# ConwayBeyond/Funscript-Flow

Hardware: AMD Instinct MI355X
Metric: 1080p frame-pairs/sec (higher is better)
Workload: dtype f32; 1 GPU; 1920x1080 synthetic sine-translate frame-pair stream, gray frames resident in HBM; levels=4, winsize=15, poly_n=5, parallelism=pair-shard x1, compute_lanes=1, kernel_signature=872b792e378b97e5

## Files before the change

### funscript_flow_amd/csrc/ffl_api.hip

```cpp
#include "../../include/ffl.h"
#include "ffl_kernels.h"

#include <math.h>
#include <stdarg.h>
#include <stdio.h>
#include <string.h>

#include <algorithm>
#include <condition_variable>
#include <mutex>
#include <string>
#include <thread>
#include <vector>

#define FFL_EV_RING 16
#define FFL_RAW_RING 4

template <class H, class Arg, hipError_t (*Free)(Arg)>
struct Owned {
    H h = H();
    Owned() = default;
    explicit Owned(H take) : h(take) {}
    Owned(Owned &&o) noexcept : h(o.release()) {}
    Owned &operator=(Owned &&o) noexcept { std::swap(h, o.h); return *this; }
// ... 1254 lines not shown
    HIPCHK(c, hipStreamSynchronize(c->s_copy));
    return FFL_OK;
}

struct DebugCapture {
    int level, iter;
    float *I0, *I1, *R0, *R1, *M, *flow;
};

static int enqueue_batch(ffl_ctx *c, ffl_ctx::Lane &L, const BatchTab &T, int n, int nU, int pov_mode, const DebugCapture *cap) {
    hipStream_t st = L.st;
    const size_t N = c->N;
    const UTab *ut = &L.d_tab->ut;
    const PairTab *pt = &L.d_tab->pt;
    const PyrJob *l0 = &L.pyr[L.n_jobs - 1];
    const bool fuse_l0 = c->opt.fuse_l0_blur && ffl_polyexp_from_gray_ok(*l0);
    const int skip_l0 = fuse_l0 && !cap;
    {
        ProfScope ps(c, FFL_K_PYRAMID, st);
        if (!ffl_launch_pyr_multi(c->d_gray, N, ut, nU, L.pyr, L.n_jobs - skip_l0, c->opt, st))
            for (int k = c->geo.levels; k >= skip_l0; k--)
                ffl_launch_pyr_level(c->d_gray, N, ut, nU, L.pyr[c->geo.levels - k], st);
    }
    {
        ProfScope ps(c, FFL_K_POLYEXP, st);
        ffl_launch_polyexp_multi(L.poly, L.n_jobs, nU, c->pc, c->d_gray, N, ut, fuse_l0 ? l0 : nullptr, st);
    }

    int pw = 0, ph = 0;
    for (int k = c->geo.levels; k >= 0; k--) {
        const LevelGeom &g = c->geo.lv[k];
        const int lw = g.lw, lh = g.lh;
        const size_t plane = (size_t)lw * lh;
        const size_t I_stride = plane, R_stride = 5 * plane, M_stride = 5 * plane;
        float *Rk = L.d_R + c->lay.r_off[k];
        if (pw == 0 && cap)
            for (int i = 0; i < n; i++) HIPCHK(c, hipMemsetAsync(T.pt.flow[k][i], 0, sizeof(float) * 2 * plane, st));
        int mi = 0;
        const bool fuse_first = c->opt.fuse_first > 0 && !cap && (long)((lw + 63) / 64) * ((lh + 15) / 16) * n >= c->opt.fuse_first;
        if (!fuse_first) {
            ProfScope ps(c, FFL_K_UPDATE_MATRICES, st);
            ffl_launch_update_matrices(Rk, R_stride, plane, pt, k, n, L.d_M[mi], M_stride, lw, lh, pw, ph, pw == 0, cap != nullptr, c->opt, st);
        }
        bool captured = false;
        auto capture = [&]() -> int {
            HIPCHK(c, hipStreamSynchronize(st));
            if (cap->I0) HIPCHK(c, hipMemcpy(cap->I0, L.d_I + c->lay.i_off[k] + (size_t)T.pt.u0[0] * I_stride, sizeof(float) * plane, hipMemcpyDeviceToHost));
            if (cap->I1) HIPCHK(c, hipMemcpy(cap->I1, L.d_I + c->lay.i_off[k] + (size_t)T.pt.u1[0] * I_stride, sizeof(float) * plane, hipMemcpyDeviceToHost));
            if (cap->R0) HIPCHK(c, hipMemcpy(cap->R0, Rk + (size_t)T.pt.u0[0] * R_stride, sizeof(float) * 5 * plane, hipMemcpyDeviceToHost));
            if (cap->R1) HIPCHK(c, hipMemcpy(cap->R1, Rk + (size_t)T.pt.u1[0] * R_stride, sizeof(float) * 5 * plane, hipMemcpyDeviceToHost));
            if (cap->M) HIPCHK(c, hipMemcpy(cap->M, L.d_M[mi], sizeof(float) * 5 * plane, hipMemcpyDeviceToHost));
            if (cap->flow) HIPCHK(c, hipMemcpy(cap->flow, T.pt.flow[k][0], sizeof(float) * 2 * plane, hipMemcpyDeviceToHost));
            captured = true;
            return FFL_OK;
        };
        for (int it = 0; it < 3; it++) {
            if (cap && cap->level == k && cap->iter == it) {
                int rc = capture();
                if (rc) return rc;
            }
            const int update = it < 2;
            {
                ProfScope ps(c, FFL_K_BLUR_SOLVE, st, it > 0 && !cap);
                if (it == 0 && fuse_first)
                    ffl_launch_blur_solve_first(L.d_M[mi ^ 1], M_stride, Rk, R_stride, plane, pt, k, n, lw, lh, pw, ph, c->opt, c->blur_slots, st);
                else
                    ffl_launch_blur_solve(L.d_M[mi], L.d_M[mi ^ 1], M_stride, Rk, R_stride, plane, pt, k, n, lw, lh,
                                          update, cap != nullptr, c->opt, c->blur_slots, st);
            }
            if (update) mi ^= 1;
        }
        if (cap && cap->level == k && !captured) {
            int rc = capture();
            if (rc) return rc;
        }
        pw = lw;
        ph = lh;
    }
    {
        ProfScope ps(c, FFL_K_PASS1, st);
        ffl_launch_pass1(pt, n, c->w, c->h, pov_mode, L.d_pkey, L.d_psum, st);
    }
    return FFL_OK;
}

static int batch_graph(ffl_ctx *c, ffl_ctx::Lane &L, const BatchTab &T, int n, int nU, int pov_mode,
                       ffl_ctx::Lane::GraphEntry **ge) {
    *ge = nullptr;
    for (auto &g : L.graphs)
        if (g.n == n && g.nU == nU && g.pov == pov_mode && g.epoch == c->opt_epoch) *ge = &g;
    if (*ge || c->graph_bad_epoch == c->opt_epoch) return FFL_OK;
    hipStream_t st = L.st;
    ffl_ctx::Lane::GraphEntry g = {n, nU, pov_mode, c->opt_epoch, Graph(), GraphExec()};
    hipError_t fail = hipStreamBeginCapture(st, hipStreamCaptureModeThreadLocal);
    if (fail == hipSuccess) {
        const int rc = enqueue_batch(c, L, T, n, nU, pov_mode, nullptr);
        fail = hipStreamEndCapture(st, g.graph.put());
        if (fail == hipSuccess && (rc != FFL_OK || !g.graph)) fail = hipErrorStreamCaptureInvalidated;
        if (fail == hipSuccess) fail = hipGraphInstantiate(g.exec.put(), g.graph, nullptr, nullptr, 0);
    }
    if (fail != hipSuccess) {
        g.exec.reset();
        g.graph.reset();
        (void)hipGetLastError();
// ... 41 lines not shown
        const size_t plane = (size_t)c->geo.lv[k].lw * c->geo.lv[k].lh;
        float *buf = ((c->geo.levels - k) & 1) ? L.d_flowB : L.d_flowA;
        for (int i = 0; i < n; i++)
            T.pt.flow[k][i] = (k == 0) ? c->d_flow + (size_t)slots[i] * 2 * N : buf + (size_t)i * 2 * plane;
    }
    for (int k = c->geo.levels + 1; k < FFL_MAX_LEVELS; k++)
        for (int i = 0; i < n; i++) T.pt.flow[k][i] = nullptr;
    for (int i = 0; i < nU; i++) c->u_of_fslot[T.ut.fslot[i]] = -1;
    *nU_out = nU;
    WaitOnce wait(st);
    for (int i = 0; i < nU; i++) HIPCHK(c, wait(c->ev_uploaded[T.ut.fslot[i]].get()));
    for (int i = 0; i < n; i++) HIPCHK(c, wait(c->ev_slot_done[slots[i]].get()));
    HIPCHK(c, hipMemcpyAsync(L.d_tab, &T, sizeof(BatchTab), hipMemcpyHostToDevice, st));

    if (fbg || dis) {
        if (fbg) {
            FbgWork wk;
            if (int rc = fbg_work(c, L, *fbg, nU, &wk)) return rc;
            ffl_launch_fb_general(&L.d_tab->ut, &L.d_tab->pt, n, nU, c->d_gray, N, c->w, c->h, *fbg, wk, st);
        } else {
            ffl_launch_dis(&L.d_tab->ut, &L.d_tab->pt, n, c->d_gray, N, L.d_M[0], *dis, st);
        }
        ProfScope ps(c, FFL_K_PASS1, st);
        ffl_launch_pass1(&L.d_tab->pt, n, c->w, c->h, pov_mode, L.d_pkey, L.d_psum, st);
    } else if (c->opt.use_graph && !cap && c->prof_mask == 0) {
        ffl_ctx::Lane::GraphEntry *ge;
        if (int rc = batch_graph(c, L, T, n, nU, pov_mode, &ge)) return rc;
        if (ge) {
            HIPCHK(c, hipGraphLaunch(ge->exec, st));
            c->graph_replayed++;
        } else if (int rc = enqueue_batch(c, L, T, n, nU, pov_mode, nullptr)) {
            return rc;
        }
    } else if (int rc = enqueue_batch(c, L, T, n, nU, pov_mode, cap)) {
        return rc;
    }
    HIPCHK(c, hipGetLastError());
    return FFL_OK;
}

static int run_batch(ffl_ctx *c, int li, int n, const int *f0, const int *f1, const int *slots, int pov_mode,
                     const DebugCapture *cap, const DisKParams *dis = nullptr, const FbgPlan *fbg = nullptr) {
    ffl_ctx::Lane &L = c->lanes[li];
    HIPCHK(c, L.ring.settle_next());
    BatchTab &T = L.h_tab[L.ring.next % FFL_EV_RING];
    int nU = 0;
    const int rc = queue_batch(c, L, T, &nU, n, f0, f1, slots, pov_mode, cap, dis, fbg);
// ... 1952 lines not shown
    if (int rc = check_flow_slots(c, fn, n, dst_slots, nullptr, "repeated among the dst slots of one call")) return rc;
    int clash = -1;
    for (int i = 0; i < n; i++) c->slot_mark[src_slots[i]] = 1;
    for (int i = 0; i < n; i++)
        if (c->slot_mark[dst_slots[i]] && dst_slots[i] != src_slots[i] && clash < 0) clash = dst_slots[i];
    for (int i = 0; i < n; i++) c->slot_mark[src_slots[i]] = 0;
    if (clash >= 0) return set_err(c, FFL_ERR_INVALID, "%s: dst flow slot %d is another item's src slot", fn, clash);
    if (!models_dev) return set_err(c, FFL_ERR_INVALID, "%s: NULL models_dev", fn);
    if (int rc = model_array_check(c, fn, "models_dev", models_dev, model_stride)) return rc;
    int all[2 * FFL_MAXB], m = 0;
    ExportTab ts, td;
    for (int i = 0; i < n; i++) all[m++] = ts.slot[i] = src_slots[i];
    for (int i = 0; i < n; i++) {
        td.slot[i] = dst_slots[i];
        if (dst_slots[i] != src_slots[i]) all[m++] = dst_slots[i];
    }
    hipStream_t cst;
    const PostRegion reg{"models_dev", models_dev, (size_t)(n - 1) * (size_t)model_stride + 48, kHostModels};
    if (int rc = post_begin(c, fn, stream, &cst, &reg, 1, m, all)) return rc;
    ffl_launch_motion_subtract(c->d_flow, c->d_res, ts, td, n, c->w, c->h, (const char *)models_dev, (long long)model_stride, c->d_ptab,
                               c->s_post);
    {
        ProfScope ps(c, FFL_K_PASS1, c->s_post);
        ffl_launch_pass1(c->d_ptab, n, c->w, c->h, pov_mode ? 1 : 0, c->d_pskey, c->d_rpsum, c->s_post);
    }
    return post_end(c, cst, m, all);
}

static int dev_flow_check(ffl_ctx *c, const char *fn, int dtype, int n, int w, int h, const ffl_dev_flow *f, int *mode,
                          size_t *bytes) {
    if (!f) return set_err(c, FFL_ERR_INVALID, "%s: NULL descriptor", fn);
    if (dtype != FFL_F32 && dtype != FFL_F16 && dtype != FFL_BF16)
        return set_err(c, FFL_ERR_INVALID, "%s: unknown dtype %d (FFL_F32 0, FFL_F16 1, FFL_BF16 2)", fn, dtype);
    if (n < 1) return set_err(c, FFL_ERR_INVALID, "%s: n = %d fields (>= 1)", fn, n);
    if (w < 2 || h < 2 || w > 32768 || h > 32768) return set_err(c, FFL_ERR_INVALID, "%s: size %dx%d outside 2..32768", fn, w, h);
    if (!f->base) return set_err(c, FFL_ERR_INVALID, "%s: NULL base", fn);
    const ptrdiff_t e = dtype == FFL_F32 ? 4 : 2, big = (ptrdiff_t)1 << 40;
    const ptrdiff_t it = f->item_stride, pitch = f->row_pitch, ps = f->pixel_stride, cs = f->channel_stride;
    if (it < 0 || pitch < 0 || ps < 0 || cs < 0)
        return set_err(c, FFL_ERR_INVALID, "%s: negative stride (item %td, row %td, pixel %td, channel %td)", fn, it, pitch, ps, cs);
    if (it > big || pitch > big || ps > big || cs > big) return set_err(c, FFL_ERR_INVALID, "%s: stride beyond 2^40", fn);
    if ((uintptr_t)f->base % e || it % e || pitch % e || ps % e || cs % e)
        return set_err(c, FFL_ERR_INVALID, "%s: misaligned: base and strides (item %td, row %td, pixel %td, channel %td) must be "
                                           "multiples of the element size %td", fn, it, pitch, ps, cs, e);
    if (ps < e) return set_err(c, FFL_ERR_INVALID, "%s: overlap: pixel stride %td below the element size %td", fn, ps, e);
    const ptrdiff_t row = (ptrdiff_t)(w - 1) * ps + e, plane = (ptrdiff_t)(h - 1) * pitch + row;
    if (pitch < row) return set_err(c, FFL_ERR_INVALID, "%s: overlap: row pitch %td too small for %d pixels %td bytes apart", fn, pitch, w, ps);
// ... 35 lines not shown
                                c->s_post);
    }
    return post_end(c, cst, n, slots);
}

int ffl_upload_flow(ffl_ctx *c, int slot, const float *src, int pov_mode) {
    if (!c) return FFL_ERR_INVALID;
    std::unique_lock<std::mutex> pl(c->post_mu);
    CtxLock lk(c->mu);
    if (!flow_slot_ok(c, slot) || !src) return set_err(c, FFL_ERR_INVALID, "ffl_upload_flow: bad arguments");
    hipStream_t st = c->s_post;
    hipEvent_t ev = c->ev_slot_done[slot].get();
    if (int rc = wait_unlocked(c, lk, &ev, 1)) return rc;
    lk.unlock();
    hipError_t se = hipStreamSynchronize(st);
    lk.lock();
    HIPCHK(c, se);
    HIPCHK(c, hipMemcpy(c->d_flow + (size_t)slot * 2 * c->N, src, sizeof(float) * 2 * c->N, hipMemcpyHostToDevice));
    c->h_ptab->flow[0][0] = c->d_flow + (size_t)slot * 2 * c->N;
    c->h_ptab->res[0] = c->d_res + slot;
    HIPCHK(c, hipMemcpyAsync(c->d_ptab, c->h_ptab, sizeof(PairTab), hipMemcpyHostToDevice, st));
    {
        ProfScope ps(c, FFL_K_PASS1, st);
        ffl_launch_pass1(c->d_ptab, 1, c->w, c->h, pov_mode, c->d_pskey, c->d_rpsum, st);
    }
    EvRef done;
    if (int rc = publish_post(c, 1, &slot, &done)) return rc;
    HIPCHK(c, hipGetLastError());
    return FFL_OK;
}

int ffl_submit_pair(ffl_ctx *c, int slot, const uint8_t *prev, const uint8_t *next, int width, int height, int channels,
                    ptrdiff_t stride_bytes, int pov_mode) {
    if (!c) return FFL_ERR_INVALID;
    if (!flow_slot_ok(c, slot) || 2 * slot + 1 >= c->n_fslots) {
        CtxLock lk(c->mu);
        return set_err(c, FFL_ERR_INVALID, "ffl_submit_pair: slot %d needs frame slots %d,%d and a flow slot", slot, 2 * slot, 2 * slot + 1);
    }
    int rc = ffl_upload_frame(c, 2 * slot, prev, width, height, channels, stride_bytes);
    if (rc) return rc;
    rc = ffl_upload_frame(c, 2 * slot + 1, next, width, height, channels, stride_bytes);
    if (rc) return rc;
    int f0 = 2 * slot, f1 = 2 * slot + 1;
    return ffl_flow_pairs(c, 1, &f0, &f1, &slot, pov_mode);
}

int ffl_sync(ffl_ctx *c) {
// ... 138 lines not shown
```

### funscript_flow_amd/csrc/ffl_kernels.h

```cpp
#pragma once
#include <hip/hip_runtime.h>
#include <limits.h>
#include <stdint.h>

#define FFL_MAXB 256
#define FFL_MAXU (2 * FFL_MAXB)
#define FFL_MAX_LEVELS 4
#define FFL_POLY_N 5
#define FFL_WIN 15
#define FFL_WIN_R 7

struct PolyConsts {
    float g[FFL_POLY_N + 1], xg[FFL_POLY_N + 1], xxg[FFL_POLY_N + 1];
    double gd[FFL_POLY_N + 1], xxgd[FFL_POLY_N + 1];
    double ig11, ig03, ig33, ig55;
};

struct GaussKernel {
    float k[32];
    int ksize;
};

struct UTab {
    int fslot[FFL_MAXU];
// ... 87 lines not shown
    int w, h;
    unsigned gx, gy, first, count;
    int from_gray;
    float gk0, gk1;
};
struct PolyJobs {
    PolyJob j[FFL_MAX_JOBS];
    int n;
};

struct FflOptions {
    int lanes = 2;
    int fuse_first = 10000;
    int use_graph = 1;
    int copy_threads = 4;
    int blur_rows = 0;
    int blur_min_wgs = 3500;
    int tile_order = 0;
    int blur_taper = 1;
    int blur_taper_pairs = 0;
    int pyr_coarse = 1;
    int fuse_l0_blur = 1;
    int fb_general = 0;
};
struct FflOptionRow {
    const char *name;
    int FflOptions::*member;
    int lo, hi;
    bool flag;
};
inline constexpr FflOptionRow kFflOptionRows[] = {
    {"lanes", &FflOptions::lanes, 1, 4, false},
    {"fuse_first", &FflOptions::fuse_first, 0, INT_MAX, false},
    {"graph", &FflOptions::use_graph, INT_MIN, INT_MAX, true},
    {"copy_threads", &FflOptions::copy_threads, 1, 16, false},
    {"blur_rows", &FflOptions::blur_rows, 0, 64, false},
    {"blur_min_wgs", &FflOptions::blur_min_wgs, 1, INT_MAX, false},
    {"tile_order", &FflOptions::tile_order, 0, 1, false},
    {"blur_taper", &FflOptions::blur_taper, 0, 1, false},
    {"blur_taper_pairs", &FflOptions::blur_taper_pairs, 0, FFL_MAXB, false},
    {"pyr_coarse", &FflOptions::pyr_coarse, INT_MIN, INT_MAX, true},
    {"fuse_l0_blur", &FflOptions::fuse_l0_blur, INT_MIN, INT_MAX, true},
    {"fb_general", &FflOptions::fb_general, 0, 1, false},
};

#define FFL_BLUR_SEGS 3
struct BlurSeg {
    int first_block, first_pair, pairs, nrb, strips;
};
struct BlurPlan {
    BlurSeg s[FFL_BLUR_SEGS];
    int n;
};
struct BlurSlots {
    int first, first_zero, update, last;
};

bool ffl_launch_pyr_multi(const uint8_t *gray_base, size_t gray_stride, const UTab *ut, int nU, const PyrJob *levels, int n,
                          const FflOptions &opt, hipStream_t st);
bool ffl_polyexp_from_gray_ok(const PyrJob &l0);
void ffl_launch_polyexp_multi(const PolyJob *levels, int n, int nU, PolyConsts pc, const uint8_t *gray_base, size_t gray_stride,
                              const UTab *ut, const PyrJob *l0, hipStream_t st);
void ffl_launch_frontend(const FrameDesc &d, uint8_t *gray, const FrontParams &p, hipStream_t st);
void ffl_launch_frontend_dev(const FrameDesc *tab, int n, uint8_t *gray_base, size_t N, const FrontParams &p, hipStream_t st);
void ffl_launch_frontend_remap(const FrameDesc &d, uint8_t *gray, const FrontParams &p, const RemapParams &r, hipStream_t st);
void ffl_launch_frontend_remap_dev(const FrameDesc *tab, int n, uint8_t *gray_base, size_t N, const FrontParams &p,
                                   const RemapParams &r, hipStream_t st);
void ffl_launch_export_flows(const float *flow, const ExportTab &tab, int n, size_t N, char *dst, long long item_stride,
                             int layout, hipStream_t st);
void ffl_launch_import_pass1(const ImportArgs &a, const ExportTab &tab, int n, int dtype, int mode, int w, int h, int pov_mode,
                             PairTab *pt, unsigned long long *pkey, double *psum, hipStream_t st);
void ffl_launch_gray(const uint8_t *bgr, uint8_t *gray, int n_pixels, hipStream_t st);
size_t ffl_pyr_tmp_floats(int w, int h, int lw);
bool ffl_pyr_level_ok(int w, int h, int lw, int lh, int ksize);
void ffl_launch_pyr_level(const uint8_t *gray_base, size_t gray_stride, const UTab *ut, int nU, const PyrJob &level,
                          hipStream_t st);
void ffl_launch_update_matrices(const float *R, size_t R_stride, size_t plane, const PairTab *pt, int level, int nB, float *M,
                                size_t M_stride, int lw, int lh, int pw, int ph, int zero_flow, int store_flow,
                                const FflOptions &opt, hipStream_t st);
void ffl_launch_blur_solve(const float *Min, float *Mout, size_t M_stride, const float *R, size_t R_stride,
                           size_t plane, const PairTab *pt, int level, int nB, int lw, int lh, int update, int store_flow,
                           const FflOptions &opt, const BlurSlots &slots, hipStream_t st);


void ffl_launch_blur_solve_first(float *Mout, size_t M_stride, const float *R, size_t R_stride, size_t plane,
                                 const PairTab *pt, int level, int nB, int lw, int lh, int pw, int ph, const FflOptions &opt,
                                 const BlurSlots &slots, hipStream_t st);
bool ffl_blur_slots(BlurSlots *out);
unsigned ffl_blur_plan(int tiles_x, int tiles_y, int nB, int slots, const FflOptions &opt, BlurPlan *plan);

#define DIS_MAX_PATCHES 4096
#define DIS_MAX_SCALES 12
struct DisKParams {
    int w, h, finest, coarsest, stride, gd_iters, vr_iters, mean_norm, spatial_prop, stripes;
    float alpha, gamma, delta;
    size_t pair_floats;
    size_t pyr_floats;
    size_t pyr_off[DIS_MAX_SCALES];
    float *dbg;
    int dbg_scale, dbg_stage;
};
void ffl_launch_dis(const UTab *ut, const PairTab *pt, int nB, const uint8_t *gray, size_t gray_stride, float *scratch,
                    const DisKParams &p, hipStream_t st);

int ffl_pass1_blocks(int w, int h);
void ffl_launch_pass1(const PairTab *pt, int nB, int w, int h, int pov_mode, unsigned long long *pkey, double *psum,
                      hipStream_t st);

#define FFL_WINDOW_MAX_RADIUS 32
struct WindowSeq {
    int slot[FFL_MAXB + 2 * FFL_WINDOW_MAX_RADIUS];
};
struct WindowItem {
    const float *flow;
    double cx, cy;
    int cut, pad;
};
struct Pass2Record {
    double dot, cx, cy;
    float mean_mag, div_val;
    int x, y, cut, pad;
};
struct AxesRecord {
    Pass2Record base;
    double tangential, shift_x, shift_y, reserved;
};
#define FFL_NAXES 4
int ffl_radial_blocks(int w, int h);
struct RadialForm {
    int nc;
// ... 244 lines not shown
    return ffl_tile_map(blockIdx.x, tiles_x, tiles_y, nB, order, b, tile_x, tile_y);
}

__host__ __device__ __forceinline__ bool ffl_blur_block(const BlurPlan &p, unsigned blk, int tiles_x, int order, int &b,
                                                        int &tile_x, int &row0, int &nrb) {
    int first = 0, pair0 = 0, pairs = p.s[0].pairs, strips = p.s[0].strips;
    nrb = p.s[0].nrb;
#pragma unroll
    for (int i = 1; i < FFL_BLUR_SEGS; i++)
        if (i < p.n && blk >= (unsigned)p.s[i].first_block) {
            first = p.s[i].first_block;
            pair0 = p.s[i].first_pair;
            pairs = p.s[i].pairs;
            strips = p.s[i].strips;
            nrb = p.s[i].nrb;
        }
    int strip_y;
    if (!ffl_tile_map(blk - first, tiles_x, strips, pairs, order, b, tile_x, strip_y)) return false;
    b += pair0;
    row0 = strip_y * nrb;
    return true;
}

#define FFL_GLOBAL __attribute__((address_space(1)))
typedef float ffl_v2f __attribute__((ext_vector_type(2), aligned(4)));
typedef float ffl_v4f __attribute__((ext_vector_type(4), aligned(4)));
__device__ __forceinline__ float2 ffl_gload2(const void *base, size_t byte_off) {
    const ffl_v2f v = *(const FFL_GLOBAL ffl_v2f *)((const char *)base + byte_off);
    return make_float2(v.x, v.y);
}
__device__ __forceinline__ float4 ffl_gload4(const void *base, size_t byte_off) {
    const ffl_v4f v = *(const FFL_GLOBAL ffl_v4f *)((const char *)base + byte_off);
    return make_float4(v.x, v.y, v.z, v.w);
}

struct __attribute__((packed, aligned(4))) ffl_f2u { float x, y; };
struct __attribute__((packed, aligned(4))) ffl_f4u { float x, y, z, w; };

template <typename T>
__device__ __forceinline__ const T *ffl_at(const float *base, unsigned idx) {
    return reinterpret_cast<const T *>(reinterpret_cast<const char *>(base) + idx * 4u);
}
template <typename T>
__device__ __forceinline__ T *ffl_at(float *base, unsigned idx) {
    return reinterpret_cast<T *>(reinterpret_cast<char *>(base) + idx * 4u);
}
// ... 90 lines not shown
```

### funscript_flow_amd/csrc/kernels_farneback.hip

```cpp
#include "ffl_kernels.h"

#include <algorithm>

__global__ __launch_bounds__(256) void k_gray(const uint8_t *__restrict__ bgr, uint8_t *__restrict__ gray, int n) {
    int i4 = (blockIdx.x * 256 + threadIdx.x) * 4;
    if (i4 + 3 < n) {
        const uint32_t *p = reinterpret_cast<const uint32_t *>(bgr + (size_t)i4 * 3);
        uint32_t a = p[0], b = p[1], c = p[2];
        uint32_t px[12] = {a & 255, (a >> 8) & 255, (a >> 16) & 255, a >> 24, b & 255, (b >> 8) & 255,
                           (b >> 16) & 255, b >> 24, c & 255, (c >> 8) & 255, (c >> 16) & 255, c >> 24};
        uint32_t o = 0;
#pragma unroll
        for (int j = 0; j < 4; j++) {
            uint32_t g = (px[j * 3] * 3735u + px[j * 3 + 1] * 19235u + px[j * 3 + 2] * 9798u + 16384u) >> 15;
            o |= g << (8 * j);
        }
        *reinterpret_cast<uint32_t *>(gray + i4) = o;
    } else {
        for (int i = i4; i < n; i++) {
            uint32_t b = bgr[(size_t)i * 3], g = bgr[(size_t)i * 3 + 1], r = bgr[(size_t)i * 3 + 2];
            gray[i] = (uint8_t)((b * 3735u + g * 19235u + r * 9798u + 16384u) >> 15);
        }
    }
}
// ... 685 lines not shown
                    if (x + e < w) out[c * plane + off + e] = o[c][e];
        }
    }
}

__global__ __launch_bounds__(256) void k_polyexp_multi(PolyJobs jobs, PolyConsts pc, const uint8_t *__restrict__ gray_base,
                                                       size_t gray_stride, const UTab *__restrict__ ut) {
    int i = 0;
#pragma unroll
    for (int t = 1; t < FFL_MAX_JOBS; t++)
        if (t < jobs.n && blockIdx.x >= jobs.j[t].first) i = t;
    const PolyJob &J = jobs.j[i];
    const unsigned t = blockIdx.x - J.first;
    if (t >= J.count) return;
    const unsigned per = J.gx * J.gy;
    const unsigned bz = t / per, r = t - bz * per, by = r / J.gx, bx = r - by * J.gx;
    const uint8_t *gimg = J.from_gray ? gray_base + (size_t)ut->fslot[bz] * gray_stride : nullptr;
    k_polyexp_body(bx, by, bz, J.I, J.I_stride, J.R, J.R_stride, J.plane, J.w, J.h, pc, gimg, J.gk0, J.gk1);
}

bool ffl_polyexp_from_gray_ok(const PyrJob &l0) { return ffl_pyr_form(l0.w, l0.h, l0.lw, l0.lh, l0.gk.ksize).kind == FFL_PYR_F1; }

void ffl_launch_polyexp_multi(const PolyJob *jobs_in, int n, int nU, PolyConsts pc, const uint8_t *gray_base, size_t gray_stride,
                              const UTab *ut, const PyrJob *l0, hipStream_t st) {
    PolyJobs jobs = {};
    unsigned total = 0;
    for (int i = 0; i < n; i++) {
        jobs.j[i] = jobs_in[i];
        jobs.j[i].gx = (jobs_in[i].w + PE_TW - 1) / PE_TW;
        jobs.j[i].gy = (jobs_in[i].h + PE_TH - 1) / PE_TH;
        jobs.j[i].first = total;
        jobs.j[i].count = jobs.j[i].gx * jobs.j[i].gy * (unsigned)nU;
        total += jobs.j[i].count;
    }
    jobs.n = n;
    if (l0) {
        jobs.j[n - 1].from_gray = 1;
        jobs.j[n - 1].gk0 = l0->gk.k[1];
        jobs.j[n - 1].gk1 = l0->gk.k[2];
    }
    hipLaunchKernelGGL(k_polyexp_multi, dim3(total), dim3(256), 0, st, jobs, pc, gray_base, gray_stride, ut);
}

__device__ __forceinline__ float2 ffl_upsample2(const float4 c0, const float4 c1, bool first0, bool first1, float a1, float b1) {
    const float a0 = 1.f - a1, b0 = 1.f - b1;
    const float2 p00 = first0 ? make_float2(c0.x, c0.y) : make_float2(c0.z, c0.w);
    const float2 p01 = first1 ? make_float2(c0.x, c0.y) : make_float2(c0.z, c0.w);
    const float2 p10 = first0 ? make_float2(c1.x, c1.y) : make_float2(c1.z, c1.w);
    const float2 p11 = first1 ? make_float2(c1.x, c1.y) : make_float2(c1.z, c1.w);
    float2 f;
    float t0 = p00.x * a0 + p01.x * a1, t1 = p10.x * a0 + p11.x * a1;
    f.x = (t0 * b0 + t1 * b1) * 2.0f;
    t0 = p00.y * a0 + p01.y * a1;
    t1 = p10.y * a0 + p11.y * a1;
    f.y = (t0 * b0 + t1 * b1) * 2.0f;
    return f;
}

template <int NR, typename Disp, typename Keep>
__device__ __forceinline__ void ffl_um_rows(const float *R0, const float *R1, float *M, size_t plane, int w, int h, int x,
                                            bool xin, int ybase, Disp disp, Keep keep) {
    struct UmRow {
// ... 27 lines not shown
        if (k + 1 < NR) nxt = issue(k + 1);
        const bool in = xin && ybase + 4 * k < h;
        const int y = min(ybase + 4 * k, h - 1);
        const unsigned o = (unsigned)y * (unsigned)w + (unsigned)x;
        if (in) keep(o, cur.f);
        float bb[5];
#pragma unroll
        for (int c = 0; c < 5; c++) bb[c] = cur.a00 * cur.t[c].x + cur.a01 * cur.t[c].y + cur.a10 * cur.u[c].x + cur.a11 * cur.u[c].y;
        float m[5];
        ffl_um_finish(cur.r0, bb, cur.inside, w, h, x, y, cur.f.x, cur.f.y, m);
        if (in) {
#pragma unroll
            for (int c = 0; c < 5; c++) *ffl_at<float>(M + c * plane, o) = m[c];
        }
        if (k + 1 < NR) cur = nxt;
    }
}

template <int MODE>
__global__ __launch_bounds__(256) void k_update_matrices(const float *__restrict__ R, size_t R_stride, size_t plane,
                                                         const PairTab *__restrict__ pt, int level,
                                                         float *__restrict__ M, size_t M_stride, int w,
                                                         int h, int pw, int ph, double usx, double usy, int store_flow,
                                                         int nB, int order) {
    int b, tile_x, tile_y;
    if (!ffl_tile_coord((w + 63) / 64, (h + 15) / 16, nB, order, b, tile_x, tile_y)) return;
    const int lx = threadIdx.x & 63, x0 = tile_x * 64, x = min(x0 + lx, w - 1);
    const bool xin = x0 + lx < w;
    const float *R0 = R + (size_t)pt->u0[b] * R_stride, *R1 = R + (size_t)pt->u1[b] * R_stride;
    float *flow = pt->flow[level][b];
    const float *pf = pt->flow[min(level + 1, FFL_MAX_LEVELS - 1)][b];
    constexpr int NR = 4;
    const int ybase = tile_y * 16 + (threadIdx.x >> 6);
    float2 f[NR];
    if (MODE == 1) {
        const bool half_scale = usx == 0.5 && usy == 0.5;
        int xa0, xa1;
        float a1;
        if (half_scale) ffl_resize_coord_half(x, pw, xa0, xa1, a1);
        else ffl_resize_coord(x, pw, usx, xa0, xa1, a1);
        const int xq = min(xa0, pw - 2);
        float4 c0[NR], c1[NR];
        float b1[NR];
#pragma unroll
        for (int k = 0; k < NR; k++) {
            int ya0, ya1;
            const int y = min(ybase + 4 * k, h - 1);
            if (half_scale) ffl_resize_coord_half(y, ph, ya0, ya1, b1[k]);
            else ffl_resize_coord(y, ph, usy, ya0, ya1, b1[k]);
// ... 4 lines not shown
        for (int k = 0; k < NR; k++) f[k] = ffl_upsample2(c0[k], c1[k], xa0 == xq, xa1 == xq, a1, b1[k]);
    } else if (MODE == 0) {
#pragma unroll
        for (int k = 0; k < NR; k++) {
            const unsigned o = (unsigned)min(ybase + 4 * k, h - 1) * (unsigned)w + (unsigned)x;
            const FFL_GLOBAL float *q = (const FFL_GLOBAL float *)flow + 2u * o;
            f[k] = make_float2(q[0], q[1]);
        }
    } else {
#pragma unroll
        for (int k = 0; k < NR; k++) f[k] = make_float2(0.f, 0.f);
    }
    ffl_um_rows<NR>(R0, R1, M + (size_t)b * M_stride, plane, w, h, x, xin, ybase, [&](int k) { return f[k]; },
                    [&](unsigned o, float2 d) {
                        if (MODE == 1 && store_flow) {
                            flow[2u * o] = d.x;
                            flow[2u * o + 1u] = d.y;
                        }
                    });
}

void ffl_launch_update_matrices(const float *R, size_t R_stride, size_t plane, const PairTab *pt, int level, int nB,
                                float *M,
                                size_t M_stride, int lw, int lh, int pw, int ph, int zero_flow, int store_flow,
                                const FflOptions &opt, hipStream_t st) {
    dim3 grid(ffl_tile_grid((lw + 63) / 64, (lh + 15) / 16, nB));
    const auto k = pw > 0 ? k_update_matrices<1> : (zero_flow ? k_update_matrices<2> : k_update_matrices<0>);
    hipLaunchKernelGGL(k, grid, dim3(256), 0, st, R, R_stride, plane, pt, level, M, M_stride, lw, lh, pw, ph,
                       pw > 0 ? (double)pw / lw : 1.0, pw > 0 ? (double)ph / lh : 1.0, pw > 0 ? store_flow : 0, nB,
                       opt.tile_order);
}

#ifndef FFL_K5_WAVES
#define FFL_K5_WAVES 4
#endif
#ifndef FFL_K5_WAVES_FIRST
#define FFL_K5_WAVES_FIRST 3
#endif
#ifndef FFL_K5_GROUP_FIRST
#define FFL_K5_GROUP_FIRST 3
#endif
#ifndef FFL_K5_GROUP
#define FFL_K5_GROUP 3
#endif

__device__ __forceinline__ void ffl_box_block16(const float (&v)[30], double (&out)[16]) {
    double s[15];
    s[14] = (double)v[14];
#pragma unroll
    for (int j = 13; j >= 0; j--) s[j] = (double)v[j] + s[j + 1];
    double p = (double)v[15];
    out[0] = s[0];
#pragma unroll
// ... 37 lines not shown
#define FFL_DRAIN_MAX 8192
__device__ unsigned long long g_drain[3][FFL_DRAIN_MAX][2];
extern "C" int ffl_debug_read_drain(unsigned long long *out) {
    return (int)hipMemcpyFromSymbol(out, HIP_SYMBOL(g_drain), sizeof(unsigned long long) * 3 * FFL_DRAIN_MAX * 2);
}
#define FFL_DRAIN(e)                                                          \
    if (w >= 1024 && tid == 0 && blockIdx.x < FFL_DRAIN_MAX) g_drain[FIRST ? 0 : UPDATE ? 1 : 2][blockIdx.x][e] = wall_clock64();
#define FFL_T(i)                                                              \
    if (FFL_STAMP_ON && tid == 0) {                                           \
        const unsigned long long t_ = __builtin_readcyclecounter();          \
        sStamp[i] += t_ - sStamp[FFL_NSTAMP];                                 \
        sStamp[FFL_NSTAMP] = t_;                                              \
    }
#else
#define FFL_T(i)
#define FFL_DRAIN(e)
#endif


template <bool UPDATE, int FIRST>
__global__ __launch_bounds__(256, FIRST ? FFL_K5_WAVES_FIRST : FFL_K5_WAVES) void k_blur_solve(
    const float *__restrict__ Min, float *__restrict__ Mout, size_t M_stride, const float *__restrict__ R, size_t R_stride,
    size_t plane, const PairTab *__restrict__ pt, int level, int w, int h, BlurPlan plan, int pw, int ph, double usx, double usy,
    int store_flow, int order) {
    constexpr int TW = 64, TH = 16, LW = TW + 2 * FFL_WIN_R, LH = TH + 2 * FFL_WIN_R;
    constexpr int PX = 4;
    constexpr int NCARRY = LH - TH;
    constexpr int LW2 = 44;
    constexpr int GC = FIRST ? FFL_K5_GROUP_FIRST : FFL_K5_GROUP, NG = (5 + GC - 1) / GC;
    __shared__ double2 sS2[GC][TH][LW2];
    const int tid = threadIdx.x;
#ifdef FFL_STAMP
    __shared__ unsigned long long sStamp[FFL_NSTAMP + 1];
    const bool FFL_STAMP_ON = FIRST == 1 && w >= 1024;
    if (FFL_STAMP_ON && tid == 0) {
        for (int i = 0; i < FFL_NSTAMP; i++) sStamp[i] = 0;
        sStamp[FFL_NSTAMP] = __builtin_readcyclecounter();
    }
#endif
    int b, tile_x, row0, nrb;
    if (!ffl_blur_block(plan, blockIdx.x, (w + TW - 1) / TW, order, b, tile_x, row0, nrb)) return;
    FFL_DRAIN(0)
    const int x0 = tile_x * TW;
    const float *Mb = Min + (size_t)b * M_stride;

    const int q = __builtin_amdgcn_readfirstlane(tid >> 6);
    const int ty = (tid & 63) >> 2, kk = tid & 3;
    const int lx0 = 16 * kk + 4 * q;
    double *sS = reinterpret_cast<double *>(&sS2[0][0][0]);
    const int vcc = tid / LW, vtx = tid - vcc * LW;
    const int vgx = min(max(x0 + vtx - FFL_WIN_R, 0), w - 1);
    const unsigned pitch = (unsigned)w * 4u;
    float carry[NG][NCARRY];
    const double scale = 1.0 / (FFL_WIN * FFL_WIN);
    float2 *flow = reinterpret_cast<float2 *>(pt->flow[level][b]);
    const float *R0 = R + (size_t)pt->u0[b] * R_stride, *R1 = R + (size_t)pt->u1[b] * R_stride;
    float *Mo = Mout + (size_t)b * M_stride;
    constexpr int FP = TW + 2;
    float4 *sF4 = reinterpret_cast<float4 *>(&sS2[0][0][0]);
    constexpr int UP = 80;
    __shared__ float sM34[FIRST ? 5 - GC : 1][FIRST ? TH : 1][FIRST ? UP : 1];
    float *sM012 = reinterpret_cast<float *>(&sS2[0][0][0]);
    static_assert(GC * TH * UP * 4 <= (int)sizeof(sS2), "the first group's staged rows must fit the column sums");
    const float2 *prevf = reinterpret_cast<const float2 *>(pt->flow[min(level + 1, FFL_MAX_LEVELS - 1)][b]);
// ... 268 lines not shown
    int per_cu = 0;
    if (hipOccupancyMaxActiveBlocksPerMultiprocessor(&per_cu, k, 256, 0) != hipSuccess) return 0;
    return per_cu * cus;
}
bool ffl_blur_slots(BlurSlots *out) {
    int dev = 0, cus = 0;
    if (hipGetDevice(&dev) != hipSuccess || hipDeviceGetAttribute(&cus, hipDeviceAttributeMultiprocessorCount, dev) != hipSuccess)
        return false;
    *out = BlurSlots{ffl_k5_slots(k_blur_solve<true, 1>, cus), ffl_k5_slots(k_blur_solve<true, 2>, cus),
                     ffl_k5_slots(k_blur_solve<true, 0>, cus), ffl_k5_slots(k_blur_solve<false, 0>, cus)};
    return out->first > 0 && out->first_zero > 0 && out->update > 0 && out->last > 0;
}
#ifdef FFL_STAMP
extern "C" int ffl_debug_blur_slots(int *out) {
    BlurSlots s;
    if (!ffl_blur_slots(&s)) return 1;
    out[0] = s.first; out[1] = s.first_zero; out[2] = s.update; out[3] = s.last;
    return 0;
}
#endif

template <typename K>
static void ffl_launch_k5(K k, const float *Min, float *Mout, size_t M_stride, const float *R, size_t R_stride, size_t plane,
                          const PairTab *pt, int level, int nB, int lw, int lh, int pw, int ph, int store_flow,
                          const FflOptions &opt, int slots, hipStream_t st) {
    BlurPlan plan;
    dim3 grid(ffl_blur_plan((lw + 63) / 64, (lh + 15) / 16, nB, slots, opt, &plan));
    hipLaunchKernelGGL(k, grid, dim3(256), 0, st, Min, Mout, M_stride, R, R_stride, plane, pt, level, lw, lh, plan, pw, ph,
                       pw > 0 ? (double)pw / lw : 1.0, pw > 0 ? (double)ph / lh : 1.0, store_flow, opt.tile_order);
}

void ffl_launch_blur_solve(const float *Min, float *Mout, size_t M_stride, const float *R, size_t R_stride,
                           size_t plane, const PairTab *pt, int level, int nB, int lw, int lh, int update, int store_flow,
                           const FflOptions &opt, const BlurSlots &slots, hipStream_t st) {
    ffl_launch_k5(update ? k_blur_solve<true, 0> : k_blur_solve<false, 0>, Min, Mout, M_stride, R, R_stride, plane, pt, level,
                  nB, lw, lh, 0, 0, update ? store_flow : 1, opt, update ? slots.update : slots.last, st);
}

void ffl_launch_blur_solve_first(float *Mout, size_t M_stride, const float *R, size_t R_stride, size_t plane,
                                 const PairTab *pt, int level, int nB, int lw, int lh, int pw, int ph, const FflOptions &opt,
                                 const BlurSlots &slots, hipStream_t st) {
    ffl_launch_k5(pw > 0 ? k_blur_solve<true, 1> : k_blur_solve<true, 2>, (const float *)nullptr, Mout, M_stride, R, R_stride,
                  plane, pt, level, nB, lw, lh, pw, ph, 0, opt, pw > 0 ? slots.first : slots.first_zero, st);
}
```

### funscript_flow_amd/csrc/kernels_post.hip

```cpp
#include "ffl_kernels.h"
#include <cassert>
#include <cfloat>
#include <type_traits>

#define P1_THREADS 256
#define P1_RG 16
#ifndef P1_G
#define P1_G 16
#endif
#define P1_STRIP 126
#define P2_STRIP 128
#ifndef P2_AXES_G
#define P2_AXES_G 2
#endif

static inline int ffl_strip_waves(int w, int h, int strip) {
    return ((w + strip - 1) / strip) * ((h + P1_RG - 1) / P1_RG);
}
int ffl_pass1_blocks(int w, int h) { return (ffl_strip_waves(w, h, P1_STRIP) + 3) / 4; }
int ffl_radial_blocks(int w, int h) { return (ffl_strip_waves(w, h, P2_STRIP) + 3) / 4; }

__device__ __forceinline__ float ffl_grad(float lo, float hi, int idx, int n) {
    return (idx == 0 || idx == n - 1) ? hi - lo : (hi - lo) / 2.0f;
}
// ... 129 lines not shown
    key = ffl_wave_max_u64(key);
    sum = ffl_wave_sum_f64(sum);
    if constexpr (Wt::on) sw = ffl_wave_sum_f64(sw);
    if (lane == 0) {
        skey[wv] = key;
        ssum[wv] = sum;
        if constexpr (Wt::on) ssw[wv] = sw;
    }
    __syncthreads();
    if (threadIdx.x == 0) {
        for (int i = 1; i < P1_THREADS / 64; i++) {
            key = skey[i] > key ? skey[i] : key;
            sum += ssum[i];
            if constexpr (Wt::on) sw += ssw[i];
        }
        pkey[(size_t)b * gridDim.x + blockIdx.x] = key;
        psum[(size_t)b * gridDim.x + blockIdx.x] = sum;
        if constexpr (Wt::on) psw[(size_t)b * gridDim.x + blockIdx.x] = sw;
    }
}

__global__ __launch_bounds__(P1_THREADS) void k_pass1(const PairTab *__restrict__ pt, int w, int h, int pov_mode,
                                                      unsigned long long *__restrict__ pkey,
                                                      double *__restrict__ psum) {
    __shared__ unsigned long long skey[P1_THREADS / 64];
    __shared__ double ssum[P1_THREADS / 64];
    const int b = blockIdx.y;
    const P1SlotSrc src{reinterpret_cast<const float2 *>(pt->flow[0][b]), w};
    ffl_pass1_body(src, WtNone{}, w, h, pov_mode, b, pkey, psum, skey, ssum);
}

template <bool WT>
__device__ __forceinline__ void ffl_pass1_final_body(const PairTab *__restrict__ pt, int w, int h, int pov_mode, int nblk,
                                                     const unsigned long long *__restrict__ pkey,
                                                     const double *__restrict__ psum, const double *__restrict__ psw,
                                                     unsigned long long *skey, double *ssum, double *ssw) {
    const int b = blockIdx.x;
    unsigned long long key = 0;
    double sum = 0.0;
    [[maybe_unused]] double sw = 0.0;
    for (int i = threadIdx.x; i < nblk; i += P1_THREADS) {
        unsigned long long k = pkey[(size_t)b * nblk + i];
        key = k > key ? k : key;
        sum += psum[(size_t)b * nblk + i];
        if constexpr (WT) sw += psw[(size_t)b * nblk + i];
    }
    key = ffl_wave_max_u64(key);
    sum = ffl_wave_sum_f64(sum);
    if constexpr (WT) sw = ffl_wave_sum_f64(sw);
    int lane = threadIdx.x & 63, wv = threadIdx.x >> 6;
// ... 22 lines not shown
            r.div_val = 0.f;
        } else {
            unsigned idx = 0xFFFFFFFFu - (unsigned)(key & 0xFFFFFFFFull);
            r.y = idx / w;
            r.x = idx - r.y * w;
            r.div_val = ffl_div_at(reinterpret_cast<const float2 *>(pt->flow[0][b]), w, h, r.x, r.y);
        }
        r.weighted = WT ? 1 : 0;
        r.mag_sum = sum;
        if constexpr (WT) r.mag_sum = empty ? 0.0 : sum / (empty ? 1.0 : sw);
        *pt->res[b] = r;
    }
}

__global__ __launch_bounds__(P1_THREADS) void k_pass1_final(const PairTab *__restrict__ pt, int w, int h, int pov_mode,
                                                            int nblk, const unsigned long long *__restrict__ pkey,
                                                            const double *__restrict__ psum) {
    __shared__ unsigned long long skey[P1_THREADS / 64];
    __shared__ double ssum[P1_THREADS / 64];
    ffl_pass1_final_body<false>(pt, w, h, pov_mode, nblk, pkey, psum, nullptr, skey, ssum, nullptr);
}

void ffl_launch_pass1(const PairTab *pt, int nB, int w, int h, int pov_mode, unsigned long long *pkey, double *psum,
                      hipStream_t st) {
    const int nblk = ffl_pass1_blocks(w, h);
    hipLaunchKernelGGL(k_pass1, dim3(nblk, nB), dim3(P1_THREADS), 0, st, pt, w, h, pov_mode, pkey, psum);
    hipLaunchKernelGGL(k_pass1_final, dim3(nB), dim3(P1_THREADS), 0, st, pt, w, h, pov_mode, nblk, pkey, psum);
}


template <int NC>
__device__ __forceinline__ void ffl_radial_terms(double (&sum)[NC], bool in, float2 f, double dx, double dy, double wx, double wy) {
    const double u = (double)f.x, v = (double)f.y;
    sum[0] += in ? (u * dx + v * dy) * wx * wy : 0.0;
    if constexpr (NC > 1) {
        sum[1] += in ? (v * dx - u * dy) * wx * wy : 0.0;
        sum[2] += in ? u * wx * wy : 0.0;
        sum[3] += in ? v * wx * wy : 0.0;
    }
}

struct NoWeights {};
__device__ __forceinline__ WtNone ffl_item_weights(const NoWeights &, int) { return WtNone{}; }
__device__ __forceinline__ WtBytes ffl_item_weights(const WeightArgs &wa, int b) {
    return WtBytes{wa.base + (long long)b * wa.item, wa.pitch};
}

template <int NS>
__device__ __forceinline__ size_t ffl_partial_index(int b, int c, int nblk, int g) {
// ... 1091 lines not shown
```

Measured before the change: 6431 pairs/s.

## Alternate pair traversal order across kernels to reuse L2/MALL-resident data

Reorders the multi-level polynomial expansion so the finest level runs first. It also reverses the pair index order on alternating launches of the update, blur-solve and pass1 kernels. Each kernel then starts on the pairs the previous kernel touched last, whose data are more likely still in cache. Both behaviours are on by default but can be turned off with new options, and they add a little index arithmetic in each kernel.

```diff
diff --git a/funscript_flow_amd/csrc/ffl_api.hip b/funscript_flow_amd/csrc/ffl_api.hip
--- a/funscript_flow_amd/csrc/ffl_api.hip
+++ b/funscript_flow_amd/csrc/ffl_api.hip
@@ -1300,11 +1300,19 @@
             for (int k = c->geo.levels; k >= skip_l0; k--)
                 ffl_launch_pyr_level(c->d_gray, N, ut, nU, L.pyr[c->geo.levels - k], st);
     }
+    const int finest_first = c->opt.poly_order && !cap;
     {
         ProfScope ps(c, FFL_K_POLYEXP, st);
-        ffl_launch_polyexp_multi(L.poly, L.n_jobs, nU, c->pc, c->d_gray, N, ut, fuse_l0 ? l0 : nullptr, st);
-    }
-
+        ffl_launch_polyexp_multi(L.poly, L.n_jobs, nU, c->pc, c->d_gray, N, ut, fuse_l0 ? l0 : nullptr, finest_first, st);
+    }
+
+    const int alternate = c->opt.pair_order && !cap;
+    int flip = alternate && finest_first;
+    auto next_flip = [&]() {
+        const int f = flip;
+        flip ^= alternate;
+        return f;
+    };
     int pw = 0, ph = 0;
     for (int k = c->geo.levels; k >= 0; k--) {
         const LevelGeom &g = c->geo.lv[k];
@@ -1318,7 +1326,7 @@
         const bool fuse_first = c->opt.fuse_first > 0 && !cap && (long)((lw + 63) / 64) * ((lh + 15) / 16) * n >= c->opt.fuse_first;
         if (!fuse_first) {
             ProfScope ps(c, FFL_K_UPDATE_MATRICES, st);
-            ffl_launch_update_matrices(Rk, R_stride, plane, pt, k, n, L.d_M[mi], M_stride, lw, lh, pw, ph, pw == 0, cap != nullptr, c->opt, st);
+            ffl_launch_update_matrices(Rk, R_stride, plane, pt, k, n, L.d_M[mi], M_stride, lw, lh, pw, ph, pw == 0, cap != nullptr, next_flip(), c->opt, st);
         }
         bool captured = false;
         auto capture = [&]() -> int {
@@ -1341,10 +1349,10 @@
             {
                 ProfScope ps(c, FFL_K_BLUR_SOLVE, st, it > 0 && !cap);
                 if (it == 0 && fuse_first)
-                    ffl_launch_blur_solve_first(L.d_M[mi ^ 1], M_stride, Rk, R_stride, plane, pt, k, n, lw, lh, pw, ph, c->opt, c->blur_slots, st);
+                    ffl_launch_blur_solve_first(L.d_M[mi ^ 1], M_stride, Rk, R_stride, plane, pt, k, n, lw, lh, pw, ph, next_flip(), c->opt, c->blur_slots, st);
                 else
                     ffl_launch_blur_solve(L.d_M[mi], L.d_M[mi ^ 1], M_stride, Rk, R_stride, plane, pt, k, n, lw, lh,
-                                          update, cap != nullptr, c->opt, c->blur_slots, st);
+                                          update, cap != nullptr, next_flip(), c->opt, c->blur_slots, st);
             }
             if (update) mi ^= 1;
         }
@@ -1357,7 +1365,7 @@
     }
     {
         ProfScope ps(c, FFL_K_PASS1, st);
-        ffl_launch_pass1(pt, n, c->w, c->h, pov_mode, L.d_pkey, L.d_psum, st);
+        ffl_launch_pass1(pt, n, c->w, c->h, pov_mode, L.d_pkey, L.d_psum, next_flip(), st);
     }
     return FFL_OK;
 }
@@ -1445,7 +1453,7 @@
             ffl_launch_dis(&L.d_tab->ut, &L.d_tab->pt, n, c->d_gray, N, L.d_M[0], *dis, st);
         }
         ProfScope ps(c, FFL_K_PASS1, st);
-        ffl_launch_pass1(&L.d_tab->pt, n, c->w, c->h, pov_mode, L.d_pkey, L.d_psum, st);
+        ffl_launch_pass1(&L.d_tab->pt, n, c->w, c->h, pov_mode, L.d_pkey, L.d_psum, 0, st);
     } else if (c->opt.use_graph && !cap && c->prof_mask == 0) {
         ffl_ctx::Lane::GraphEntry *ge;
         if (int rc = batch_graph(c, L, T, n, nU, pov_mode, &ge)) return rc;
@@ -3444,7 +3452,7 @@
                                c->s_post);
     {
         ProfScope ps(c, FFL_K_PASS1, c->s_post);
-        ffl_launch_pass1(c->d_ptab, n, c->w, c->h, pov_mode ? 1 : 0, c->d_pskey, c->d_rpsum, c->s_post);
+        ffl_launch_pass1(c->d_ptab, n, c->w, c->h, pov_mode ? 1 : 0, c->d_pskey, c->d_rpsum, 0, c->s_post);
     }
     return post_end(c, cst, m, all);
 }
@@ -3526,7 +3534,7 @@
     HIPCHK(c, hipMemcpyAsync(c->d_ptab, c->h_ptab, sizeof(PairTab), hipMemcpyHostToDevice, st));
     {
         ProfScope ps(c, FFL_K_PASS1, st);
-        ffl_launch_pass1(c->d_ptab, 1, c->w, c->h, pov_mode, c->d_pskey, c->d_rpsum, st);
+        ffl_launch_pass1(c->d_ptab, 1, c->w, c->h, pov_mode, c->d_pskey, c->d_rpsum, 0, st);
     }
     EvRef done;
     if (int rc = publish_post(c, 1, &slot, &done)) return rc;
diff --git a/funscript_flow_amd/csrc/ffl_kernels.h b/funscript_flow_amd/csrc/ffl_kernels.h
--- a/funscript_flow_amd/csrc/ffl_kernels.h
+++ b/funscript_flow_amd/csrc/ffl_kernels.h
@@ -133,6 +133,8 @@
     int pyr_coarse = 1;
     int fuse_l0_blur = 1;
     int fb_general = 0;
+    int pair_order = 1;
+    int poly_order = 1;
 };
 struct FflOptionRow {
     const char *name;
@@ -153,6 +155,8 @@
     {"pyr_coarse", &FflOptions::pyr_coarse, INT_MIN, INT_MAX, true},
     {"fuse_l0_blur", &FflOptions::fuse_l0_blur, INT_MIN, INT_MAX, true},
     {"fb_general", &FflOptions::fb_general, 0, 1, false},
+    {"pair_order", &FflOptions::pair_order, 0, 1, false},
+    {"poly_order", &FflOptions::poly_order, 0, 1, false},
 };
 
 #define FFL_BLUR_SEGS 3
@@ -171,7 +175,7 @@
                           const FflOptions &opt, hipStream_t st);
 bool ffl_polyexp_from_gray_ok(const PyrJob &l0);
 void ffl_launch_polyexp_multi(const PolyJob *levels, int n, int nU, PolyConsts pc, const uint8_t *gray_base, size_t gray_stride,
-                              const UTab *ut, const PyrJob *l0, hipStream_t st);
+                              const UTab *ut, const PyrJob *l0, int finest_first, hipStream_t st);
 void ffl_launch_frontend(const FrameDesc &d, uint8_t *gray, const FrontParams &p, hipStream_t st);
 void ffl_launch_frontend_dev(const FrameDesc *tab, int n, uint8_t *gray_base, size_t N, const FrontParams &p, hipStream_t st);
 void ffl_launch_frontend_remap(const FrameDesc &d, uint8_t *gray, const FrontParams &p, const RemapParams &r, hipStream_t st);
@@ -187,16 +191,16 @@
 void ffl_launch_pyr_level(const uint8_t *gray_base, size_t gray_stride, const UTab *ut, int nU, const PyrJob &level,
                           hipStream_t st);
 void ffl_launch_update_matrices(const float *R, size_t R_stride, size_t plane, const PairTab *pt, int level, int nB, float *M,
-                                size_t M_stride, int lw, int lh, int pw, int ph, int zero_flow, int store_flow,
+                                size_t M_stride, int lw, int lh, int pw, int ph, int zero_flow, int store_flow, int flip,
                                 const FflOptions &opt, hipStream_t st);
 void ffl_launch_blur_solve(const float *Min, float *Mout, size_t M_stride, const float *R, size_t R_stride,
                            size_t plane, const PairTab *pt, int level, int nB, int lw, int lh, int update, int store_flow,
-                           const FflOptions &opt, const BlurSlots &slots, hipStream_t st);
+                           int flip, const FflOptions &opt, const BlurSlots &slots, hipStream_t st);
 
 
 void ffl_launch_blur_solve_first(float *Mout, size_t M_stride, const float *R, size_t R_stride, size_t plane,
-                                 const PairTab *pt, int level, int nB, int lw, int lh, int pw, int ph, const FflOptions &opt,
-                                 const BlurSlots &slots, hipStream_t st);
+                                 const PairTab *pt, int level, int nB, int lw, int lh, int pw, int ph, int flip,
+                                 const FflOptions &opt, const BlurSlots &slots, hipStream_t st);
 bool ffl_blur_slots(BlurSlots *out);
 unsigned ffl_blur_plan(int tiles_x, int tiles_y, int nB, int slots, const FflOptions &opt, BlurPlan *plan);
 
@@ -216,7 +220,7 @@
 
 int ffl_pass1_blocks(int w, int h);
 void ffl_launch_pass1(const PairTab *pt, int nB, int w, int h, int pov_mode, unsigned long long *pkey, double *psum,
-                      hipStream_t st);
+                      int flip, hipStream_t st);
 
 #define FFL_WINDOW_MAX_RADIUS 32
 struct WindowSeq {
@@ -507,6 +511,15 @@
     return true;
 }
 
+__host__ __device__ __forceinline__ int ffl_pair_flip(int p, int n, int flip) { return flip ? n - 1 - p : p; }
+__host__ __device__ __forceinline__ int ffl_blur_plan_pairs(const BlurPlan &p) {
+    int n = p.s[0].pairs;
+#pragma unroll
+    for (int i = 1; i < FFL_BLUR_SEGS; i++)
+        if (i < p.n) n += p.s[i].pairs;
+    return n;
+}
+
 #define FFL_GLOBAL __attribute__((address_space(1)))
 typedef float ffl_v2f __attribute__((ext_vector_type(2), aligned(4)));
 typedef float ffl_v4f __attribute__((ext_vector_type(4), aligned(4)));
diff --git a/funscript_flow_amd/csrc/kernels_farneback.hip b/funscript_flow_amd/csrc/kernels_farneback.hip
--- a/funscript_flow_amd/csrc/kernels_farneback.hip
+++ b/funscript_flow_amd/csrc/kernels_farneback.hip
@@ -731,22 +731,24 @@
 bool ffl_polyexp_from_gray_ok(const PyrJob &l0) { return ffl_pyr_form(l0.w, l0.h, l0.lw, l0.lh, l0.gk.ksize).kind == FFL_PYR_F1; }
 
 void ffl_launch_polyexp_multi(const PolyJob *jobs_in, int n, int nU, PolyConsts pc, const uint8_t *gray_base, size_t gray_stride,
-                              const UTab *ut, const PyrJob *l0, hipStream_t st) {
+                              const UTab *ut, const PyrJob *l0, int finest_first, hipStream_t st) {
     PolyJobs jobs = {};
     unsigned total = 0;
     for (int i = 0; i < n; i++) {
-        jobs.j[i] = jobs_in[i];
-        jobs.j[i].gx = (jobs_in[i].w + PE_TW - 1) / PE_TW;
-        jobs.j[i].gy = (jobs_in[i].h + PE_TH - 1) / PE_TH;
+        const PolyJob &in = jobs_in[finest_first ? n - 1 - i : i];
+        jobs.j[i] = in;
+        jobs.j[i].gx = (in.w + PE_TW - 1) / PE_TW;
+        jobs.j[i].gy = (in.h + PE_TH - 1) / PE_TH;
         jobs.j[i].first = total;
         jobs.j[i].count = jobs.j[i].gx * jobs.j[i].gy * (unsigned)nU;
         total += jobs.j[i].count;
     }
     jobs.n = n;
     if (l0) {
-        jobs.j[n - 1].from_gray = 1;
-        jobs.j[n - 1].gk0 = l0->gk.k[1];
-        jobs.j[n - 1].gk1 = l0->gk.k[2];
+        PolyJob &j0 = jobs.j[finest_first ? 0 : n - 1];
+        j0.from_gray = 1;
+        j0.gk0 = l0->gk.k[1];
+        j0.gk1 = l0->gk.k[2];
     }
     hipLaunchKernelGGL(k_polyexp_multi, dim3(total), dim3(256), 0, st, jobs, pc, gray_base, gray_stride, ut);
 }
@@ -820,9 +822,10 @@
                                                          const PairTab *__restrict__ pt, int level,
                                                          float *__restrict__ M, size_t M_stride, int w,
                                                          int h, int pw, int ph, double usx, double usy, int store_flow,
-                                                         int nB, int order) {
+                                                         int nB, int order, int flip) {
     int b, tile_x, tile_y;
     if (!ffl_tile_coord((w + 63) / 64, (h + 15) / 16, nB, order, b, tile_x, tile_y)) return;
+    b = ffl_pair_flip(b, nB, flip);
     const int lx = threadIdx.x & 63, x0 = tile_x * 64, x = min(x0 + lx, w - 1);
     const bool xin = x0 + lx < w;
     const float *R0 = R + (size_t)pt->u0[b] * R_stride, *R1 = R + (size_t)pt->u1[b] * R_stride;
@@ -873,13 +876,13 @@
 
 void ffl_launch_update_matrices(const float *R, size_t R_stride, size_t plane, const PairTab *pt, int level, int nB,
                                 float *M,
-                                size_t M_stride, int lw, int lh, int pw, int ph, int zero_flow, int store_flow,
+                                size_t M_stride, int lw, int lh, int pw, int ph, int zero_flow, int store_flow, int flip,
                                 const FflOptions &opt, hipStream_t st) {
     dim3 grid(ffl_tile_grid((lw + 63) / 64, (lh + 15) / 16, nB));
     const auto k = pw > 0 ? k_update_matrices<1> : (zero_flow ? k_update_matrices<2> : k_update_matrices<0>);
     hipLaunchKernelGGL(k, grid, dim3(256), 0, st, R, R_stride, plane, pt, level, M, M_stride, lw, lh, pw, ph,
                        pw > 0 ? (double)pw / lw : 1.0, pw > 0 ? (double)ph / lh : 1.0, pw > 0 ? store_flow : 0, nB,
-                       opt.tile_order);
+                       opt.tile_order, flip);
 }
 
 #ifndef FFL_K5_WAVES
@@ -963,7 +966,7 @@
 __global__ __launch_bounds__(256, FIRST ? FFL_K5_WAVES_FIRST : FFL_K5_WAVES) void k_blur_solve(
     const float *__restrict__ Min, float *__restrict__ Mout, size_t M_stride, const float *__restrict__ R, size_t R_stride,
     size_t plane, const PairTab *__restrict__ pt, int level, int w, int h, BlurPlan plan, int pw, int ph, double usx, double usy,
-    int store_flow, int order) {
+    int store_flow, int order, int flip) {
     constexpr int TW = 64, TH = 16, LW = TW + 2 * FFL_WIN_R, LH = TH + 2 * FFL_WIN_R;
     constexpr int PX = 4;
     constexpr int NCARRY = LH - TH;
@@ -981,6 +984,7 @@
 #endif
     int b, tile_x, row0, nrb;
     if (!ffl_blur_block(plan, blockIdx.x, (w + TW - 1) / TW, order, b, tile_x, row0, nrb)) return;
+    b = ffl_pair_flip(b, ffl_blur_plan_pairs(plan), flip);
     FFL_DRAIN(0)
     const int x0 = tile_x * TW;
     const float *Mb = Min + (size_t)b * M_stride;
@@ -1295,24 +1299,24 @@
 
 template <typename K>
 static void ffl_launch_k5(K k, const float *Min, float *Mout, size_t M_stride, const float *R, size_t R_stride, size_t plane,
-                          const PairTab *pt, int level, int nB, int lw, int lh, int pw, int ph, int store_flow,
+                          const PairTab *pt, int level, int nB, int lw, int lh, int pw, int ph, int store_flow, int flip,
                           const FflOptions &opt, int slots, hipStream_t st) {
     BlurPlan plan;
     dim3 grid(ffl_blur_plan((lw + 63) / 64, (lh + 15) / 16, nB, slots, opt, &plan));
     hipLaunchKernelGGL(k, grid, dim3(256), 0, st, Min, Mout, M_stride, R, R_stride, plane, pt, level, lw, lh, plan, pw, ph,
-                       pw > 0 ? (double)pw / lw : 1.0, pw > 0 ? (double)ph / lh : 1.0, store_flow, opt.tile_order);
+                       pw > 0 ? (double)pw / lw : 1.0, pw > 0 ? (double)ph / lh : 1.0, store_flow, opt.tile_order, flip);
 }
 
 void ffl_launch_blur_solve(const float *Min, float *Mout, size_t M_stride, const float *R, size_t R_stride,
                            size_t plane, const PairTab *pt, int level, int nB, int lw, int lh, int update, int store_flow,
-                           const FflOptions &opt, const BlurSlots &slots, hipStream_t st) {
+                           int flip, const FflOptions &opt, const BlurSlots &slots, hipStream_t st) {
     ffl_launch_k5(update ? k_blur_solve<true, 0> : k_blur_solve<false, 0>, Min, Mout, M_stride, R, R_stride, plane, pt, level,
-                  nB, lw, lh, 0, 0, update ? store_flow : 1, opt, update ? slots.update : slots.last, st);
+                  nB, lw, lh, 0, 0, update ? store_flow : 1, flip, opt,update ? slots.update : slots.last, st);
 }
 
 void ffl_launch_blur_solve_first(float *Mout, size_t M_stride, const float *R, size_t R_stride, size_t plane,
-                                 const PairTab *pt, int level, int nB, int lw, int lh, int pw, int ph, const FflOptions &opt,
-                                 const BlurSlots &slots, hipStream_t st) {
+                                 const PairTab *pt, int level, int nB, int lw, int lh, int pw, int ph, int flip,
+                                 const FflOptions &opt, const BlurSlots &slots, hipStream_t st) {
     ffl_launch_k5(pw > 0 ? k_blur_solve<true, 1> : k_blur_solve<true, 2>, (const float *)nullptr, Mout, M_stride, R, R_stride,
-                  plane, pt, level, nB, lw, lh, pw, ph, 0, opt, pw > 0 ? slots.first : slots.first_zero, st);
-}
+                  plane, pt, level, nB, lw, lh, pw, ph, 0, flip, opt, pw > 0 ? slots.first : slots.first_zero, st);
+}
diff --git a/funscript_flow_amd/csrc/kernels_post.hip b/funscript_flow_amd/csrc/kernels_post.hip
--- a/funscript_flow_amd/csrc/kernels_post.hip
+++ b/funscript_flow_amd/csrc/kernels_post.hip
@@ -175,10 +175,10 @@
 
 __global__ __launch_bounds__(P1_THREADS) void k_pass1(const PairTab *__restrict__ pt, int w, int h, int pov_mode,
                                                       unsigned long long *__restrict__ pkey,
-                                                      double *__restrict__ psum) {
+                                                      double *__restrict__ psum, int flip) {
     __shared__ unsigned long long skey[P1_THREADS / 64];
     __shared__ double ssum[P1_THREADS / 64];
-    const int b = blockIdx.y;
+    const int b = ffl_pair_flip(blockIdx.y, gridDim.y, flip);
     const P1SlotSrc src{reinterpret_cast<const float2 *>(pt->flow[0][b]), w};
     ffl_pass1_body(src, WtNone{}, w, h, pov_mode, b, pkey, psum, skey, ssum);
 }
@@ -247,9 +247,9 @@
 }
 
 void ffl_launch_pass1(const PairTab *pt, int nB, int w, int h, int pov_mode, unsigned long long *pkey, double *psum,
-                      hipStream_t st) {
+                      int flip, hipStream_t st) {
     const int nblk = ffl_pass1_blocks(w, h);
-    hipLaunchKernelGGL(k_pass1, dim3(nblk, nB), dim3(P1_THREADS), 0, st, pt, w, h, pov_mode, pkey, psum);
+    hipLaunchKernelGGL(k_pass1, dim3(nblk, nB), dim3(P1_THREADS), 0, st, pt, w, h, pov_mode, pkey, psum, flip);
     hipLaunchKernelGGL(k_pass1_final, dim3(nB), dim3(P1_THREADS), 0, st, pt, w, h, pov_mode, nblk, pkey, psum);
 }
 
```

New measurement: 6454 pairs/s (median of 5 runs). Within noise of the previous version (+0.4%).
